# LiMeng95/MultiPoseNet.pytorch

Hardware: AMD Instinct MI355X
Metric: images/sec (train fwd+bwd) ResNet101 480x480 bs=32/GPU (higher is better)
Workload: dtype bf16; 1 GPU; R101 full posenet (keypoint+detection) train step: fwd + MSE/focal losses + bwd + Adam, 480x480, 32 images/GPU, bf16 MFMA / fp32 accumulate / fp32 master weights; global_batch=32, parallelism=dp1, loss_log=asynchronous (set_lazy_log), launch=recorded launch list re-issued per step (replay.py), 87 replays, optimizer_update=Adam in one launch after backward

## Files before the change

include/mpn.h:

```cpp
#ifndef MPN_H_
#define MPN_H_
#include <stdint.h>

#ifdef __cplusplus
extern "C" {
#endif

#define MPN_F32 0
#define MPN_BF16 1
#define MPN_F16 2

#define MPN_E_BADARG (-2)
#define MPN_E_UNSUPPORTED (-3)

typedef struct MpnConvParams {
    const void* x;
    const void* w;
    void* y;
    const float* bias;
    const float* scale;
    const void* res;
    const uint8_t* res_mask;
    float* stats;
    int64_t x_sB, x_sH, x_sW;
// ... 82 lines not shown
int mpn_conv_wgrad_kernel_name(const MpnWgradParams* p, char* buf, int cap);

int mpn_reduce_partials(const float* ws, int chunks, int64_t n, float* dst, int accumulate, void* stream);

int mpn_cast_f32_to_bf16(const float* src, void* dst, int64_t n, void* stream);
int mpn_cast_f32(const float* src, void* dst, int64_t n, int dtype, void* stream);
int mpn_weight_transpose(const float* w, void* wt, int Cout, int RS, int Cin, int Cout_pad,
                         int dtype, void* stream);
int mpn_weight_transpose_batched(const float* arena, void* dst, const int64_t* table, int nlayers, int64_t nblocks,
                                 int dtype, void* stream);
int mpn_weight_pad_k(const float* w, void* dst, int Cout, int K, int Kpad, int dtype, void* stream);
int mpn_stem_pack_weight(const float* w, void* packed, int Cout, int dtype, void* stream);
int mpn_stem_unpack_wgrad(const float* dpacked, float* dw, int Cout, void* stream);
int mpn_stem_pack_image(const float* img, int64_t sB, int64_t sC, int64_t sH, int64_t sW, void* dst,
                        int B, int H, int W, int dtype, void* stream);

int mpn_bn_finalize_train(const float* stats, int tiles, int C, int64_t count, const float* gamma,
                          const float* beta, float* running_mean, float* running_var, float momentum,
                          float eps, float* mean, float* invstd, float* scale, float* shift, void* stream);
int mpn_bn_finalize_eval(int C, const float* gamma, const float* beta, const float* running_mean,
                         const float* running_var, float eps, float* mean, float* invstd,
                         float* scale, float* shift, void* stream);
int mpn_bn_act_forward(const void* y, const void* res, void* z, const float* scale, const float* shift,
                       int64_t P, int C, int Cs, int relu, int dtype, uint8_t* mask, void* stream);
int mpn_bn_bwd_reduce(const void* dz, const void* z, const void* y, const float* mean, const float* invstd,
                      const float* mask_scale, const float* mask_shift, float* partial, int chunks, int64_t P, int C, int Cs, int relu, int dtype, void* stream);
int mpn_bn_bwd_finalize(const float* partial, int chunks, int C, int64_t count, const float* gamma, const float* mean,
                        const float* invstd, int train, float* dgamma, float* dbeta, float* coef, void* stream);
int mpn_bn_bwd_apply(const void* dz, const void* z, const void* y, const float* k1, const float* k2, const float* k3,
                     const float* mask_scale, const float* mask_shift, void* dy, void* dres, int dres_accumulate, int64_t P, int C, int Cs, int relu, int dtype,
                     const uint8_t* mask, void* stream);
int mpn_bn_bwd_chunks(int64_t P, int Cs, int dtype);

int mpn_maxpool3x3s2_forward(const void* x, void* y, uint8_t* idx, int B, int H, int W, int Cs,
                             int Ho, int Wo, int dtype, void* stream);
int mpn_maxpool3x3s2_backward(const void* dy, const uint8_t* idx, void* dx, int B, int H, int W, int Cs,
                              int Ho, int Wo, int dtype, void* stream);
int mpn_upsample_nearest_backward(const void* dfine, void* dcoarse, int B, int Hf, int Wf, int Hc, int Wc,
                                  int Cs, int accumulate, int dtype, void* stream);
int mpn_upsample_nearest_slice(const void* src, void* dst, int B, int Hs, int Ws, int Cs_src,
                               int Ho, int Wo, int Cs_dst, int c_off, int dtype, void* stream);
int mpn_upsample_nearest_slice_backward(const void* ddst, void* dsrc, int B, int Hs, int Ws, int Cs_src,
                                        int Ho, int Wo, int Cs_dst, int c_off, int dtype, void* stream);
int mpn_export_f32(const void* src, int src_dtype, float* dst, int B, int Hs, int Ws, int Cs, int C,
                   int Ho, int Wo, int64_t dst_sB, int64_t dst_sP, void* stream);
int mpn_import_grad(const float* ddst, int64_t ddst_sB, int64_t ddst_sP, void* dsrc, int dst_dtype,
                    int B, int Hs, int Ws, int Cs, int C, int Ho, int Wo, void* stream);
int mpn_nchw_to_nhwc_f32(const float* src, int64_t sB, int64_t sC, int64_t sH, int64_t sW, float* dst,
                         int B, int C, int H, int W, void* stream);
int mpn_det_pack(const void* src, int src_dtype, float* dst, int B, int64_t HW, int Cs, int C, int64_t dst_sB, void* stream);
int mpn_det_unpack(const float* ddst, void* dsrc, int dst_dtype, int B, int64_t HW, int Cs, int C, int64_t dst_sB, void* stream);
int mpn_relu_forward(const void* x, void* y, int64_t n, int dtype, void* stream);
int mpn_relu_backward(const void* dz, const void* z, void* dx, int64_t n, int accumulate, int dtype, void* stream);
int mpn_add_inplace(void* dst, const void* src, int64_t n, int dtype, void* stream);
int mpn_channel_sum(const void* dy, int dy_dtype, int64_t P, int C, int Cs, float* partial, int chunks, void* stream);
int mpn_channel_sum_chunks(int64_t P, int Cs, int dtype);
int mpn_colsum_rows(const void* dy, int dy_dtype, int64_t P, int C, int Cs, float* db, void* stream);

int mpn_mse_heatmap_forward(const float* const* preds, const int64_t* pred_sP, const float* gt, const float* wgt,
                            int64_t npix, float* partial, int chunks, float* out, void* stream);
int mpn_mse_heatmap_backward(const float* const* preds, float* const* dpreds, const int64_t* pred_sP,
                             const int64_t* dpred_sP, const int32_t* pred_C, const float* gt, const float* wgt,
                             int64_t npix, const float* gscale, void* stream);
int mpn_mse_chunks(int64_t npix);
int mpn_mse_train_blocks(int B, int H, int W);
int mpn_mse_heatmap_train(const float* const* levels, void* const* dlevels, const int32_t* level_Cs, int dtype,
// ... 131 lines not shown
```

multiposenet/pytorch_amd/_lib.py:

```python
import ctypes
import os
import subprocess

import torch

_HERE = os.path.dirname(os.path.abspath(__file__))
LIB_PATH = os.path.join(_HERE, "libmpn_hip.so")
CSRC = os.path.join(_HERE, "csrc")

F32, BF16, F16 = 0, 1, 2


class MpnError(RuntimeError):
    pass


class ConvParams(ctypes.Structure):
    _fields_ = [
        ("x", ctypes.c_void_p), ("w", ctypes.c_void_p), ("y", ctypes.c_void_p),
        ("bias", ctypes.c_void_p), ("scale", ctypes.c_void_p), ("res", ctypes.c_void_p), ("res_mask", ctypes.c_void_p),
        ("stats", ctypes.c_void_p),
        ("x_sB", ctypes.c_int64), ("x_sH", ctypes.c_int64), ("x_sW", ctypes.c_int64),
        ("y_sB", ctypes.c_int64), ("y_sP", ctypes.c_int64),
        ("res_sB", ctypes.c_int64), ("res_sP", ctypes.c_int64),
# ... 45 lines not shown
    "mpn_resize": (_i, [_vp, _i64, _i64, _i64, _i, _i, _i, _vp, _i, _i, _i, ctypes.c_double, ctypes.c_double, _vp]),
    "mpn_prn_build_maps": (_i, [_vp, _vp, _vp, _vp, _i, _i, _i, ctypes.c_double, _vp, _vp, _vp, _vp, _vp]),
    "mpn_prn_scores": (_i, [_vp, _vp, _i, _i, _i, _i, _vp, _vp, _vp]),
    "mpn_prn_scores_compact": (_i, [_vp, _vp, _i, _i, _i, _i, _i, _vp, _vp, _vp, _vp, _vp, _vp]),
    "mpn_prn_match_host": (_i, [_i, _vp, _vp, _vp, _vp, _vp, _vp, _vp, _i, _vp, _i, _i, _vp, _vp]),
    "mpn_conv_stats_tiles": (_i, [_PC]),
    "mpn_conv_kernel_name": (_i, [_PC, ctypes.c_char_p, _i]),
    "mpn_conv_forward": (_i, [_PC, _vp]),
    "mpn_debug_wgrad_prof": (_i, [_vp]),
    "mpn_debug_igemm_prof": (_i, [_vp]),
    "mpn_conv_wgrad_chunks": (_i, [_PW]),
    "mpn_conv_wgrad_seg_plan": (_i, [_PW]),
    "mpn_conv_wgrad": (_i, [_PW, _vp]),
    "mpn_conv_wgrad_partials": (_i, [_PW, _vp]),
    "mpn_conv_wgrad_reduce": (_i, [_PW, _vp]),
    "mpn_conv_wgrad_kernel_id": (_i, [_PW]),
    "mpn_conv_wgrad_kernel_name": (_i, [_PW, ctypes.c_char_p, _i]),
    "mpn_reduce_partials": (_i, [_vp, _i, _i64, _vp, _i, _vp]),
    "mpn_cast_f32_to_bf16": (_i, [_vp, _vp, _i64, _vp]),
    "mpn_cast_f32": (_i, [_vp, _vp, _i64, _i, _vp]),
    "mpn_weight_transpose": (_i, [_vp, _vp, _i, _i, _i, _i, _i, _vp]),
    "mpn_weight_transpose_batched": (_i, [_vp, _vp, _vp, _i, _i64, _i, _vp]),
    "mpn_weight_pad_k": (_i, [_vp, _vp, _i, _i, _i, _i, _vp]),
    "mpn_stem_pack_weight": (_i, [_vp, _vp, _i, _i, _vp]),
    "mpn_stem_unpack_wgrad": (_i, [_vp, _vp, _i, _vp]),
    "mpn_stem_pack_image": (_i, [_vp, _i64, _i64, _i64, _i64, _vp, _i, _i, _i, _i, _vp]),
    "mpn_bn_finalize_train": (_i, [_vp, _i, _i, _i64, _vp, _vp, _vp, _vp, _f, _f, _vp, _vp, _vp, _vp, _vp]),
    "mpn_bn_finalize_eval": (_i, [_i, _vp, _vp, _vp, _vp, _f, _vp, _vp, _vp, _vp, _vp]),
    "mpn_bn_act_forward": (_i, [_vp, _vp, _vp, _vp, _vp, _i64, _i, _i, _i, _i, _vp, _vp]),
    "mpn_bn_bwd_reduce": (_i, [_vp, _vp, _vp, _vp, _vp, _vp, _vp, _vp, _i, _i64, _i, _i, _i, _i, _vp]),
    "mpn_bn_bwd_finalize": (_i, [_vp, _i, _i, _i64, _vp, _vp, _vp, _i, _vp, _vp, _vp, _vp]),
    "mpn_bn_bwd_apply": (_i, [_vp, _vp, _vp, _vp, _vp, _vp, _vp, _vp, _vp, _vp, _i, _i64, _i, _i, _i, _i, _vp, _vp]),
    "mpn_bn_bwd_chunks": (_i, [_i64, _i, _i]),
    "mpn_maxpool3x3s2_forward": (_i, [_vp, _vp, _vp, _i, _i, _i, _i, _i, _i, _i, _vp]),
    "mpn_maxpool3x3s2_backward": (_i, [_vp, _vp, _vp, _i, _i, _i, _i, _i, _i, _i, _vp]),
    "mpn_upsample_nearest_backward": (_i, [_vp, _vp, _i, _i, _i, _i, _i, _i, _i, _i, _vp]),
    "mpn_upsample_nearest_slice": (_i, [_vp, _vp, _i, _i, _i, _i, _i, _i, _i, _i, _i, _vp]),
    "mpn_upsample_nearest_slice_backward": (_i, [_vp, _vp, _i, _i, _i, _i, _i, _i, _i, _i, _i, _vp]),
    "mpn_export_f32": (_i, [_vp, _i, _vp, _i, _i, _i, _i, _i, _i, _i, _i64, _i64, _vp]),
    "mpn_import_grad": (_i, [_vp, _i64, _i64, _vp, _i, _i, _i, _i, _i, _i, _i, _i, _vp]),
    "mpn_nchw_to_nhwc_f32": (_i, [_vp, _i64, _i64, _i64, _i64, _vp, _i, _i, _i, _i, _vp]),
    "mpn_det_pack": (_i, [_vp, _i, _vp, _i, _i64, _i, _i, _i64, _vp]),
    "mpn_det_unpack": (_i, [_vp, _vp, _i, _i, _i64, _i, _i, _i64, _vp]),
    "mpn_relu_forward": (_i, [_vp, _vp, _i64, _i, _vp]),
    "mpn_relu_backward": (_i, [_vp, _vp, _vp, _i64, _i, _i, _vp]),
    "mpn_add_inplace": (_i, [_vp, _vp, _i64, _i, _vp]),
    "mpn_channel_sum": (_i, [_vp, _i, _i64, _i, _i, _vp, _i, _vp]),
    "mpn_colsum_rows": (_i, [_vp, _i, _i64, _i, _i, _vp, _vp]),
    "mpn_channel_sum_chunks": (_i, [_i64, _i, _i]),
    "mpn_mse_chunks": (_i, [_i64]),
    "mpn_mse_heatmap_forward": (_i, [_vp, _vp, _vp, _vp, _i64, _vp, _i, _vp, _vp]),
    "mpn_mse_heatmap_backward": (_i, [_vp, _vp, _vp, _vp, _vp, _vp, _vp, _i64, _vp, _vp]),
    "mpn_mse_train_blocks": (_i, [_i, _i, _i]),
    "mpn_mse_heatmap_train": (_i, [_vp, _vp, _vp, _i, _vp, _vp, _i64, _i64, _i64, _i, _i, _i, _vp, _vp, _i, _vp, _vp]),
    "mpn_focal_blocks": (_i, [_i]),
    "mpn_focal_forward": (_i, [_vp, _vp, _vp, _vp, _i, _i, _i, _vp, _vp, _vp, _vp]),
    "mpn_focal_backward": (_i, [_vp, _vp, _vp, _vp, _i, _i, _i, _vp, _vp, _vp, _vp, _vp]),
    "mpn_focal_mc_blocks": (_i, [_i]),
    "mpn_focal_forward_mc": (_i, [_vp, _vp, _vp, _vp, _i, _i, _i, _i, _vp, _vp, _vp, _vp, _vp]),
    "mpn_focal_backward_mc": (_i, [_vp, _vp, _vp, _vp, _i, _i, _i, _i, _vp, _vp, _vp, _vp, _vp]),
    "mpn_class_max": (_i, [_vp, _i, _i, _i, _vp, _vp, _vp]),
    "mpn_sigmoid_forward": (_i, [_vp, _vp, _i64, _vp]),
    "mpn_gather_dets": (_i, [_vp, _vp, _i, _vp, _vp, _vp]),
    "mpn_sigmoid_backward": (_i, [_vp, _vp, _vp, _i64, _vp]),
    "mpn_add_softmax_rows": (_i, [_vp, _i64, _vp, _vp, _i, _i, _i, _vp]),
    "mpn_softmax_rows_backward": (_i, [_vp, _vp, _vp, _i64, _vp, _i, _i, _vp]),
# ... 113 lines not shown
```

multiposenet/pytorch_amd/csrc/bn.hip:

```cpp
#include "common.h"
#include <stdlib.h>

namespace {

template <typename T> struct Geo {
    static constexpr int V = Vec16<T>::N;
    int G, GB, lanes, g, pl, c0;
    __device__ __forceinline__ Geo(int Cs) {
        G = Cs / V;
        GB = G < 256 ? G : 256;
        lanes = 256 / GB;
        g = blockIdx.y * GB + (threadIdx.x % GB);
        pl = threadIdx.x / GB;
        c0 = g * V;
    }
};

template <int V>
__device__ __forceinline__ void load_coef(const float* __restrict__ p, int c0, int C, float (&out)[V], float fill) {
#pragma unroll
    for (int k = 0; k < V; k += 4) {
        if (p != nullptr && c0 + k + 3 < C) {
            const float4 t = *reinterpret_cast<const float4*>(p + c0 + k);
            out[k] = t.x; out[k + 1] = t.y; out[k + 2] = t.z; out[k + 3] = t.w;
// ... 211 lines not shown
    load_coef<V>(k3p, q.c0, C, k3, 0.f);
    const bool bits = relu && mask != nullptr;
    const bool remask = relu && !bits && z == nullptr;
    float sc[V], sf[V];
    if (remask) { load_coef<V>(mscale, q.c0, C, sc, 0.f); load_coef<V>(mshift, q.c0, C, sf, 0.f); }
    const bool need_y = ((dy != nullptr) && (k2p != nullptr)) || remask;
    const long p0 = (long)blockIdx.x * q.lanes * iters + q.pl;
    for (int it = 0; it < iters; ++it) {
        const long p = p0 + (long)it * q.lanes;
        if (p >= P) break;
        const long off = p * Cs + q.c0;
        Vec16<T> d, o, x, out, r;
        d.load(dz + off);
        if (need_y) x.load(y + off);
        if (relu && !remask && !bits) o.load(z + off);
        unsigned mb = 0;
        if (bits) mb = mask[p * q.G + q.g];
        if (dres && dres_acc) r.load(dres + off);
#pragma unroll
        for (int k = 0; k < V; ++k) {
            float gk = d.v[k];
            if (remask) o.v[k] = x.v[k] * sc[k] + sf[k];
            if (bits) o.v[k] = ((mb >> k) & 1u) ? 1.f : 0.f;
            if (relu && !(o.v[k] > 0.f)) gk = 0.f;
            const bool live = q.c0 + k < C;
            out.v[k] = live ? (k1[k] * gk + (k2p ? k2[k] * x.v[k] : 0.f) + k3[k]) : 0.f;
            if (dres) r.v[k] = (dres_acc ? r.v[k] : 0.f) + (live ? gk : 0.f);
        }
        if (dy) out.store(dy + off);
        if (dres) r.store(dres + off);
    }
}

inline int geo_lanes(int Cs, int V) { const int G = Cs / V; return 256 / (G < 256 ? G : 256); }
inline int geo_yblocks(int Cs, int V) { const int G = Cs / V; return G <= 256 ? 1 : G / 256; }
inline bool geo_ok(int Cs, int V) { const int G = Cs / V; return Cs % V == 0 && G > 0 && (G & (G - 1)) == 0; }

inline int pick_iters(long P, int lanes) {
    static const long blocks = mpn_tune("MPN_BN_BLOCKS", 8192);
    long it = P / ((long)lanes * blocks);
    if (it < 1) it = 1;
    if (it > 32) it = 32;
    return (int)it;
}
inline int reduce_chunk(long P, int lanes) {
    long c = P / 512;
    const long lo = (long)lanes * 4, hi = 4096;
    if (c < lo) c = lo;
    if (c > hi) c = hi;
    return (int)((c + lanes - 1) / lanes * lanes);
}

}

extern "C" int mpn_bn_finalize_train(const float* stats, int tiles, int C, int64_t count, const float* gamma,
                                     const float* beta, float* running_mean, float* running_var, float momentum,
                                     float eps, float* mean, float* invstd, float* scale, float* shift, void* stream) {
    MPN_CHECK_ARG(stats && tiles > 0 && C > 0 && count > 0 && mean && invstd && scale && shift);
    hipLaunchKernelGGL(bn_finalize_train_kernel, dim3((C + 3) / 4), dim3(256), 0, (hipStream_t)stream, stats, tiles, C,
                       (double)count, gamma, beta, running_mean, running_var, momentum, eps, mean, invstd, scale, shift);
    return mpn_launch_status();
}

extern "C" int mpn_bn_finalize_eval(int C, const float* gamma, const float* beta, const float* running_mean,
                                    const float* running_var, float eps, float* mean, float* invstd,
                                    float* scale, float* shift, void* stream) {
// ... 31 lines not shown
    const int chunk = reduce_chunk(P, geo_lanes(Cs, V));
    MPN_CHECK_ARG(chunks == (int)((P + chunk - 1) / chunk));
    dim3 grid((unsigned)chunks, (unsigned)geo_yblocks(Cs, V));
    MPN_DISPATCH_T(dtype, hipLaunchKernelGGL((bn_bwd_reduce_kernel<T>), grid, dim3(256), 0, (hipStream_t)stream, (const T*)dz, (const T*)z,
                           (const T*)y, mean, invstd, mask_scale, mask_shift, partial, (long)P, C, Cs, relu, chunk));
    return mpn_launch_status();
}

extern "C" int mpn_bn_bwd_finalize(const float* partial, int chunks, int C, int64_t count, const float* gamma, const float* mean,
                                   const float* invstd, int train, float* dgamma, float* dbeta, float* coef, void* stream) {
    MPN_CHECK_ARG(partial && chunks > 0 && C > 0 && count > 0);
    MPN_CHECK_ARG(!coef || (mean && invstd));
    hipLaunchKernelGGL(bn_bwd_finalize_kernel, dim3((C + 3) / 4), dim3(256), 0, (hipStream_t)stream, partial, chunks, C,
                       (double)count, gamma, mean, invstd, train, dgamma, dbeta, coef);
    return mpn_launch_status();
}

extern "C" int mpn_bn_bwd_apply(const void* dz, const void* z, const void* y, const float* k1, const float* k2, const float* k3,
                                const float* mask_scale, const float* mask_shift, void* dy, void* dres, int dres_accumulate, int64_t P, int C, int Cs, int relu, int dtype,
                                const uint8_t* mask, void* stream) {
    MPN_CHECK_ARG(dz && (dy || dres) && P > 0 && C > 0 && Cs >= C);
    MPN_CHECK_ARG(!dy || k1);
    MPN_CHECK_ARG(!(dy && k2) || y);
    MPN_CHECK_ARG(!relu || z || mask || (mask_scale && mask_shift && y));
    const int V = dtype == MPN_F32 ? 4 : 8;
    MPN_CHECK_ARG(geo_ok(Cs, V) && C % 4 == 0);
    const int lanes = geo_lanes(Cs, V), iters = pick_iters(P, lanes);
    dim3 grid((unsigned)((P + (long)lanes * iters - 1) / ((long)lanes * iters)), (unsigned)geo_yblocks(Cs, V));
    MPN_DISPATCH_T(dtype, hipLaunchKernelGGL((bn_bwd_apply_kernel<T>), grid, dim3(256), 0, (hipStream_t)stream, (const T*)dz, (const T*)z,
                           (const T*)y, k1, k2, k3, mask_scale, mask_shift, (T*)dy, (T*)dres, dres_accumulate, (long)P, C, Cs, relu, iters,
                           (const unsigned char*)mask));
    return mpn_launch_status();
}
```

multiposenet/pytorch_amd/engine.py:

```python
import ctypes
import os

import torch

from . import ops
from ._lib import MpnError, call, gpu_op
from .ops import Act, round_up


class Ctx(object):

    def __init__(self, train):
        self.train = train
        self.tape = []
        self.grads = {}
        self.keep = []
        self.out_grads = {}
        self.wt = {}
        self.wt_buf = None
        self.uses = {}
        self.bn_train_ran = False
        self.side_keep = []
        self.wt_ready = None
        self.bnb = {}
# ... 22 lines not shown
        return self.grads.pop(id(act), None)


def num_classes(cm):
    cout = cm.output.weight.shape[0]
    if cout % 9 != 0 or cout == 0 or getattr(cm, "num_anchors", 9) != 9:
        raise MpnError("classificationModel: the output convolution has %d channels; the detector needs 9 anchors x K classes" % cout)
    return cout // 9


def _geom(layer):
    w = layer.weight
    if w.dim() == 2:
        return w.shape[0], w.shape[1], 1, 1, 1, 0
    return w.shape[0], w.shape[1], w.shape[2], w.shape[3], layer.stride[0], layer.padding[0]


class Engine(object):
    def __init__(self, model):
        self.m = model
        self._drop_calls = 0
        self._side = None
        self._wt_plan_cache = None
        self.overlap_wgrad = os.environ.get("MPN_SIDE_STREAM", "1") != "0"
        self.pyramid_towers = os.environ.get("MPN_PYRAMID_TOWERS", "1") != "0"
        self.fuse_bn_stats = os.environ.get("MPN_BN_FUSED_STATS", "1") != "0"
        self.fold_bn = os.environ.get("MPN_FOLD_BN", "1") != "0"
        self.fuse_bn_finalize = os.environ.get("MPN_BN_FUSED_FINALIZE", "1") != "0"
        self.det_pyramid_side = int(os.environ.get("MPN_DET_PYRAMID_SIDE", "2"))
        self.bn_mask_bits = os.environ.get("MPN_BN_MASK_BITS", "1") != "0"
        self.defer_shortcut_grad = os.environ.get("MPN_DEFER_SHORTCUT_GRAD", "1") != "0"
        self.virtual_concat = os.environ.get("MPN_VIRTUAL_CONCAT", "1") != "0"
        self.conv2_classes = os.environ.get("MPN_CONV2_CLASSES", "1") != "0"

    def side_stream(self, device):
        if not self.overlap_wgrad or device.type != "cuda":
            return None
        if self._side is None:
            self._side = torch.cuda.Stream(device=device)
        return self._side

    def _on_side(self, ctx, device, keep, fn, torch_ops=False, done_event=False):
        side = self.side_stream(device)
        if side is None:
            fn()
            return None
        ctx.side_keep.append(keep)
        ev = torch.cuda.Event()
        gpu_op(ev.record, torch.cuda.current_stream(device))
        gpu_op(side.wait_event, ev)
        if torch_ops:
            with torch.cuda.stream(side):
                fn()
        else:
            ops.push_stream(side)
            try:
                fn()
            finally:
                ops.pop_stream()
        if not done_event:
            return None
        done = torch.cuda.Event()
        gpu_op(done.record, side)
        return done

    @property
# ... 221 lines not shown
            raise MpnError("pyramid convolution: gradient missing for some levels")
        if act == 1:
            fd, fy = ops.seg_flat(dys), ops.seg_flat(ys)
            if fd is not None and fy is not None and fd.numel() == fy.numel():
                out = ops.alloc_seg(ys, ys[0].C, dys[0].t.dtype)
                call("mpn_relu_backward", ops.ptr(fd), ops.ptr(fy), ops.ptr(out[0].seg[0]), fy.numel(), 0, ops.dtype_code(fy.dtype), ops.stream_ptr())
                dys = out
            else:
                dys = [ops.relu_backward(d, y) for d, y in zip(dys, ys)]
        pyr = []

        def wgrad(dw, db, i):
            if i == 0:
                pyr[:] = ops.conv_wgrad_seg(xs, dys, dw, O, R, S, pad, db=db)
            return pyr[1] if pyr[0] else ops.conv_wgrad(xs[i], dys[i], dw, O, R, S, 1, pad, db=db)
        self._param_grads(ctx, layer, dys, (xs, dys), wgrad)
        if any(x.needs_grad for x in xs):
            wt = self.w_t(ctx, layer)
            grouped = ops.seg_flat(xs) is not None
            if grouped and ctx.grad_of(xs[0]) is None:
                gs = ops.alloc_seg(xs, xs[0].C, xs[0].t.dtype)
                for x, g in zip(xs, gs):
                    ctx.set_grad(x, g)
                existed = [False] * len(xs)
            else:
                pairs = [ctx.gbuf(x) for x in xs]
                gs, existed = [g for g, _ in pairs], [e for _, e in pairs]
            if all(existed) or not any(existed):
                ops.conv_forward_seg(dys, wt, I, R, S, pad, mode=1, cin=wt.shape[3], outs=gs, accumulate=existed[0])
            else:
                for d, x, g, e in zip(dys, xs, gs, existed):
                    ops.conv_forward(d, wt, I, R, S, 1, pad, mode=1, out_hw=(x.H, x.W), cin=wt.shape[3], out=g, accumulate=e)

    def bn(self, ctx, y, stats, layer, relu, res=None, tag=""):
        train_stats = layer.training
        want_mask = bool(self.bn_mask_bits and ctx.train and relu and res is not None)
        if train_stats:
            momentum = layer.momentum if layer.momentum is not None else 0.1
            if isinstance(stats, ops.BNState):
                st = stats
            else:
                st = ops.bn_finalize_train(stats, y.P, layer.weight.data, layer.bias.data, layer.running_mean, layer.running_var,
                                           momentum, layer.eps)
            ctx.bn_train_ran = True
        else:
            st = ops.bn_finalize_eval(layer.weight.data, layer.bias.data, layer.running_mean, layer.running_var, layer.eps)
        z = ops.bn_act(y, st, relu, res=res, tag=tag, want_mask=want_mask)
        if ctx.train:
            z.needs_grad = bool(y.needs_grad or layer.weight.requires_grad or layer.bias.requires_grad
                                or (res is not None and res.needs_grad))
            if z.needs_grad:
                self._note_use(ctx, layer.weight)
                self._note_use(ctx, layer.bias)
                if res is not None and res.needs_grad:
                    res.cons += 1
                    res.other_cons += 1
                wants_stats = bool(train_stats or layer.weight.requires_grad or layer.bias.requires_grad)
                z.bn_src = (y, st, relu, res is not None, wants_stats, layer, train_stats)
                ctx.tape.append(lambda: self._bn_bwd(ctx, y, z, st, layer, relu, res, train_stats))
        return z

    @staticmethod
    def _bnb_args(fused):
        if fused is None:
            return {}
        if isinstance(fused, str) or (fused.dim() == 2 and fused.shape[0] == 3):
            return {"coef": fused}
        return {"partial": fused}

    def _bn_bwd(self, ctx, y, z, st, layer, relu, res, train_stats):
        dz = ctx.pop_grad(z)
        wg, bg = layer.weight.requires_grad, layer.bias.requires_grad
        if dz is None:
            self._param_grads(ctx, layer, None)
            if res is not None and res.needs_grad:
                res.cons -= 1
            return
        ar = self.m._arena
        dres, dres_acc = None, False
# ... 260 lines not shown
            img = img.float()
        packed = torch.empty((B, Hp, Wp, 4), dtype=self.cdt, device=img.device)
        call("mpn_stem_pack_image", ops.ptr(img), img.stride(0), img.stride(1), img.stride(2), img.stride(3), ops.ptr(packed),
             B, H, W, ops.dtype_code(self.cdt), ops.stream_ptr())
        xa = Act(packed, 4)
        w = f.conv1.weight
        wp = torch.empty((64, 7, 32), dtype=self.cdt, device=img.device)
        call("mpn_stem_pack_weight", ops.ptr(self.m._arena.data_seg(w)), ops.ptr(wp), 64, ops.dtype_code(self.cdt), ops.stream_ptr())
        Ho, Wo = ops.conv_out_hw(H, W, 7, 7, 2, 3)
        geom = (Hp, Wp, Hp * Wp * 4, Wp * 4, 4)
        bn_train = f.bn1.training
        if self.fold_bn and not ctx.train and not bn_train:
            bst = ops.bn_finalize_eval(f.bn1.weight.data, f.bn1.bias.data, f.bn1.running_mean, f.bn1.running_var, f.bn1.eps)
            z, _ = ops.conv_forward(xa, wp, 64, 7, 1, 2, 0, cin=32, x_geom=geom, out_hw=(Ho, Wo), scale=bst.scale, bias=bst.shift, act=1)
            return self.maxpool(ctx, z)
        y, st = ops.conv_forward(xa, wp, 64, 7, 1, 2, 0, cin=32, x_geom=geom, out_hw=(Ho, Wo), want_stats=bn_train,
                                 bn_fin=self._bn_fin(f.bn1) if bn_train else None)
        if ctx.train and w.requires_grad:
            y.needs_grad = True
            self._note_use(ctx, w)

            def bwd():
                dy = ctx.pop_grad(y)
                if dy is None:
                    return self._param_grads(ctx, f.conv1, None)
                dwp = torch.empty((64, 7, 32), dtype=torch.float32, device=img.device)

                def wgrad(dw, db, i):
                    call("mpn_fill_f32", ops.ptr(dwp), 0.0, dwp.numel(), ops.stream_ptr())
                    ops.conv_wgrad(xa, dy, dwp, 64, 7, 1, 2, 0, cin=32, x_geom=geom)
                    call("mpn_stem_unpack_wgrad", ops.ptr(dwp), ops.ptr(dw), 64, ops.stream_ptr())
                self._param_grads(ctx, f.conv1, (dy,), (xa, dy, dwp), wgrad)
            ctx.tape.append(bwd)
        z = self.bn(ctx, y, st, f.bn1, True)
        return self.maxpool(ctx, z)

    def conv_bn(self, ctx, x, conv, bn, relu, res=None):
        if self.fold_bn and not ctx.train and not bn.training:
            st = ops.bn_finalize_eval(bn.weight.data, bn.bias.data, bn.running_mean, bn.running_var, bn.eps)
            O, I, R, S, stride, pad = _geom(conv)
            act = (3 if res is not None else 1) if relu else 0
            y, _ = ops.conv_forward(x, self.w_fwd(conv), O, R, S, stride, pad, scale=st.scale, bias=st.shift, act=act,
                                    res=res, res_mode=1 if res is not None else 0)
            return y
        y, s = self.conv(ctx, x, conv, stats=bn.training, bn=bn)
        return self.bn(ctx, y, s, bn, relu, res=res)

    def bottleneck(self, ctx, x, blk):
        z1 = self.conv_bn(ctx, x, blk.conv1, blk.bn1, True)
        z2 = self.conv_bn(ctx, z1, blk.conv2, blk.bn2, True)
        sc = self.conv_bn(ctx, x, blk.downsample[0], blk.downsample[1], False) if len(blk.downsample) > 0 else x
        return self.conv_bn(ctx, z2, blk.conv3, blk.bn3, True, res=sc)

    def backbone(self, ctx, img):
        f = self.m.fpn
        c = self.stem(ctx, img)
        feats = []
        for layer in (f.layer1, f.layer2, f.layer3, f.layer4):
            for blk in layer:
                c = self.bottleneck(ctx, c, blk)
            feats.append(c)
        return feats

    def det_pyramid(self, ctx, c3, c4, c5):
        f = self.m.fpn

        def coarse(h):
            h["p6"], _ = self.conv(ctx, c5, f.conv6)
# ... 160 lines not shown
```

multiposenet/pytorch_amd/ops.py:

```python
import ctypes
import os

import torch

from . import _lib
from ._lib import BF16, F16, F32, ConvParams, WgradParams, call


def round_up(v, m):
    return (v + m - 1) // m * m


def dtype_code(dt):
    if dt == torch.float32:
        return F32
    if dt == torch.bfloat16:
        return BF16
    if dt == torch.float16:
        return F16
    raise _lib.MpnError("unsupported dtype %s" % dt)


_STREAM_OVERRIDE = []

# ... 665 lines not shown
                 chunks, P, C, Cs, 1 if relu else 0, dc, stream_ptr())
        coef = torch.empty((3, C), dtype=torch.float32, device=dev) if train else None
        call("mpn_bn_bwd_finalize", ptr(part), chunks, C, P, ptr(gamma), ptr(st.mean), ptr(st.invstd), 1 if train else 0,
             ptr(dgamma), ptr(dbeta), ptr(coef), stream_ptr())
        if train:
            k1, k2, k3 = coef[0], coef[1], coef[2]
    dy = None
    if want_dy or dres is not None:
        if want_dy:
            dy = Act(torch.empty_like(y.t), C)
        bits = z.mask if (relu and not remask) else None
        call("mpn_bn_bwd_apply", ptr(dz.t), ptr(z.t) if (relu and not remask and bits is None) else None, ptr(y.t), ptr(k1), ptr(k2), ptr(k3),
             ptr(st.scale) if remask else None, ptr(st.shift) if remask else None,
             ptr(dy.t) if dy is not None else None, ptr(dres.t) if dres is not None else None,
             1 if dres_acc else 0, P, C, Cs, 1 if relu else 0, dc, ptr(bits), stream_ptr())
    return dy


def maxpool_forward(x, needs_grad=False):
    Ho, Wo = (x.H + 2 - 3) // 2 + 1, (x.W + 2 - 3) // 2 + 1
    y = Act(torch.empty((x.B, Ho, Wo, x.Cs), dtype=x.t.dtype, device=x.t.device), x.C, needs_grad)
    idx = torch.empty((x.B, Ho, Wo, x.Cs), dtype=torch.uint8, device=x.t.device) if needs_grad else None
    call("mpn_maxpool3x3s2_forward", ptr(x.t), ptr(y.t), ptr(idx), x.B, x.H, x.W, x.Cs, Ho, Wo, dtype_code(x.t.dtype), stream_ptr())
    return y, idx


def maxpool_backward(dy, idx, x_like):
    dx = Act(torch.empty_like(x_like.t), x_like.C)
    call("mpn_maxpool3x3s2_backward", ptr(dy.t), ptr(idx), ptr(dx.t), x_like.B, x_like.H, x_like.W, x_like.Cs, dy.H, dy.W,
         dtype_code(dy.t.dtype), stream_ptr())
    return dx


def upsample_backward(dfine, dcoarse, accumulate):
    call("mpn_upsample_nearest_backward", ptr(dfine.t), ptr(dcoarse.t), dfine.B, dfine.H, dfine.W, dcoarse.H, dcoarse.W,
         dfine.Cs, 1 if accumulate else 0, dtype_code(dfine.t.dtype), stream_ptr())


def upsample_slice(src, dst, c_off):
    call("mpn_upsample_nearest_slice", ptr(src.t), ptr(dst.t), src.B, src.H, src.W, src.Cs, dst.H, dst.W, dst.Cs, c_off,
         dtype_code(src.t.dtype), stream_ptr())


def upsample_slice_backward(ddst, dsrc, c_off):
    call("mpn_upsample_nearest_slice_backward", ptr(ddst.t), ptr(dsrc.t), dsrc.B, dsrc.H, dsrc.W, dsrc.Cs, ddst.H, ddst.W,
         ddst.Cs, c_off, dtype_code(dsrc.t.dtype), stream_ptr())


def export_f32(src, C, Ho, Wo):
    out = torch.empty((src.B, Ho, Wo, C), dtype=torch.float32, device=src.t.device)
    call("mpn_export_f32", ptr(src.t), dtype_code(src.t.dtype), ptr(out), src.B, src.H, src.W, src.Cs, C, Ho, Wo,
         Ho * Wo * C, C, stream_ptr())
    return out.permute(0, 3, 1, 2)


def import_grad(g_nchw, like, dtype):
    B, C, Ho, Wo = g_nchw.shape
    g = g_nchw.permute(0, 2, 3, 1)
    if g.stride(3) != 1 or g.stride(1) != Wo * g.stride(2):
        g = g.contiguous()
    d = Act(torch.empty((like.B, like.H, like.W, like.Cs), dtype=dtype, device=like.t.device), like.C)
    call("mpn_import_grad", ptr(g), g.stride(0), g.stride(2), ptr(d.t), dtype_code(dtype), like.B, like.H, like.W, like.Cs,
         like.C, Ho, Wo, stream_ptr())
    return d


# ... 163 lines not shown
```

Measured before the change: 889.8 images/sec.

## Fuse stem BN+ReLU with 3x3 maxpool in forward and backward

Adds kernels that apply the stem BatchNorm affine and ReLU while computing the 3x3/s2 maxpool, so the full-resolution post-BN activation is never written. The backward pass scatters pooled gradients through the stored argmax indices inside the BN backward reduce and apply kernels, which removes the separate maxpool backward and its full-resolution gradient tensor. This cuts several full-resolution memory passes at 240x240x64. In exchange the forward recomputes BN for overlapping pool windows, and the backward gathers up to four pooled neighbours per pixel and re-derives the ReLU mask from y and the BN coefficients.

```diff
diff --git a/include/mpn.h b/include/mpn.h
--- a/include/mpn.h
+++ b/include/mpn.h
@@ -138,6 +138,17 @@
                      const uint8_t* mask, void* stream);
 int mpn_bn_bwd_chunks(int64_t P, int Cs, int dtype);
 
+int mpn_stem_bn_act_pool_forward(const void* y, void* pooled, uint8_t* idx, uint8_t* mask, const float* scale,
+                                 const float* shift, int B, int H, int W, int C, int Cs, int Ho, int Wo, int dtype,
+                                 void* stream);
+int mpn_stem_pool_bn_bwd_reduce(const void* dpooled, const uint8_t* idx, const void* y, const float* mean,
+                                const float* invstd, const float* mask_scale, const float* mask_shift,
+                                const uint8_t* mask, float* partial, int chunks, int B, int H, int W, int C, int Cs,
+                                int Ho, int Wo, int dtype, void* stream);
+int mpn_stem_pool_bn_bwd_apply(const void* dpooled, const uint8_t* idx, const void* y, const float* k1, const float* k2,
+                               const float* k3, const float* mask_scale, const float* mask_shift, const uint8_t* mask,
+                               void* dy, int B, int H, int W, int C, int Cs, int Ho, int Wo, int dtype, void* stream);
+
 int mpn_maxpool3x3s2_forward(const void* x, void* y, uint8_t* idx, int B, int H, int W, int Cs,
                              int Ho, int Wo, int dtype, void* stream);
 int mpn_maxpool3x3s2_backward(const void* dy, const uint8_t* idx, void* dx, int B, int H, int W, int Cs,
diff --git a/multiposenet/pytorch_amd/_lib.py b/multiposenet/pytorch_amd/_lib.py
--- a/multiposenet/pytorch_amd/_lib.py
+++ b/multiposenet/pytorch_amd/_lib.py
@@ -101,6 +101,9 @@
     "mpn_bn_bwd_finalize": (_i, [_vp, _i, _i, _i64, _vp, _vp, _vp, _i, _vp, _vp, _vp, _vp]),
     "mpn_bn_bwd_apply": (_i, [_vp, _vp, _vp, _vp, _vp, _vp, _vp, _vp, _vp, _vp, _i, _i64, _i, _i, _i, _i, _vp, _vp]),
     "mpn_bn_bwd_chunks": (_i, [_i64, _i, _i]),
+    "mpn_stem_bn_act_pool_forward": (_i, [_vp, _vp, _vp, _vp, _vp, _vp, _i, _i, _i, _i, _i, _i, _i, _i, _vp]),
+    "mpn_stem_pool_bn_bwd_reduce": (_i, [_vp, _vp, _vp, _vp, _vp, _vp, _vp, _vp, _vp, _i, _i, _i, _i, _i, _i, _i, _i, _i, _vp]),
+    "mpn_stem_pool_bn_bwd_apply": (_i, [_vp, _vp, _vp, _vp, _vp, _vp, _vp, _vp, _vp, _vp, _i, _i, _i, _i, _i, _i, _i, _i, _vp]),
     "mpn_maxpool3x3s2_forward": (_i, [_vp, _vp, _vp, _i, _i, _i, _i, _i, _i, _i, _vp]),
     "mpn_maxpool3x3s2_backward": (_i, [_vp, _vp, _vp, _i, _i, _i, _i, _i, _i, _i, _vp]),
     "mpn_upsample_nearest_backward": (_i, [_vp, _vp, _i, _i, _i, _i, _i, _i, _i, _i, _vp]),
diff --git a/multiposenet/pytorch_amd/csrc/bn.hip b/multiposenet/pytorch_amd/csrc/bn.hip
--- a/multiposenet/pytorch_amd/csrc/bn.hip
+++ b/multiposenet/pytorch_amd/csrc/bn.hip
@@ -267,6 +267,227 @@
     }
 }
 
+
+template <int V> struct IdxVec;
+template <> struct IdxVec<8> {
+    uint2 t;
+    __device__ __forceinline__ void load(const uint8_t* p) { t = *reinterpret_cast<const uint2*>(p); }
+    __device__ __forceinline__ void store(uint8_t* p) const { *reinterpret_cast<uint2*>(p) = t; }
+    __device__ __forceinline__ unsigned get(int k) const { return ((k < 4 ? t.x : t.y) >> ((k & 3) * 8)) & 0xffu; }
+    __device__ __forceinline__ void set(const int (&b)[8]) {
+        t.x = (unsigned)b[0] | ((unsigned)b[1] << 8) | ((unsigned)b[2] << 16) | ((unsigned)b[3] << 24);
+        t.y = (unsigned)b[4] | ((unsigned)b[5] << 8) | ((unsigned)b[6] << 16) | ((unsigned)b[7] << 24);
+    }
+};
+template <> struct IdxVec<4> {
+    unsigned t;
+    __device__ __forceinline__ void load(const uint8_t* p) { t = *reinterpret_cast<const unsigned*>(p); }
+    __device__ __forceinline__ void store(uint8_t* p) const { *reinterpret_cast<unsigned*>(p) = t; }
+    __device__ __forceinline__ unsigned get(int k) const { return (t >> (k * 8)) & 0xffu; }
+    __device__ __forceinline__ void set(const int (&b)[4]) {
+        t = (unsigned)b[0] | ((unsigned)b[1] << 8) | ((unsigned)b[2] << 16) | ((unsigned)b[3] << 24);
+    }
+};
+
+template <typename T>
+__global__ void __launch_bounds__(256) stem_bn_act_pool_fwd_kernel(const T* __restrict__ y, T* __restrict__ out, uint8_t* __restrict__ idx,
+                                                                   unsigned char* __restrict__ mask, const float* __restrict__ scale,
+                                                                   const float* __restrict__ shift, int B, int H, int W, int C, int Cs,
+                                                                   int Ho, int Wo) {
+    constexpr int V = Vec16<T>::N;
+    const unsigned G = Cs / V;
+    const unsigned i = blockIdx.x * blockDim.x + threadIdx.x;
+    if (i >= (unsigned)B * Ho * Wo * G) return;
+    const unsigned g = i % G;
+    unsigned pix = i / G;
+    const int wo = (int)(pix % Wo); pix /= Wo;
+    const int ho = (int)(pix % Ho);
+    const int b = (int)(pix / Ho);
+    const int c0 = g * V;
+    float sc[V], sf[V];
+    load_coef<V>(scale, c0, C, sc, 0.f);
+    load_coef<V>(shift, c0, C, sf, 0.f);
+    float best[V]; int bi[V];
+#pragma unroll
+    for (int k = 0; k < V; ++k) { best[k] = -INFINITY; bi[k] = 0; }
+    bool first = true;
+    for (int r = 0; r < 3; ++r) {
+        const int h = ho * 2 - 1 + r;
+        if ((unsigned)h >= (unsigned)H) continue;
+        for (int s = 0; s < 3; ++s) {
+            const int w = wo * 2 - 1 + s;
+            if ((unsigned)w >= (unsigned)W) continue;
+            const long p = ((long)b * H + h) * W + w;
+            Vec16<T> a; a.load(y + p * Cs + c0);
+            unsigned bits = 0;
+#pragma unroll
+            for (int k = 0; k < V; ++k) {
+                float x = a.v[k] * sc[k] + sf[k];
+                x = fmaxf(x, 0.f);
+                const float v = Elem<T>::round((c0 + k < C) ? x : 0.f);
+                bits |= (v > 0.f ? 1u : 0u) << k;
+                if (first || v > best[k]) { best[k] = v; bi[k] = r * 3 + s; }
+            }
+            first = false;
+            if (mask && r >= 1 && s >= 1) mask[p * G + g] = (unsigned char)bits;
+        }
+    }
+    Vec16<T> o;
+#pragma unroll
+    for (int k = 0; k < V; ++k) o.v[k] = best[k];
+    o.store(out + (long)i * V);
+    if (idx) {
+        IdxVec<V> t; t.set(bi);
+        t.store(idx + (long)i * V);
+    }
+}
+
+template <typename T>
+struct StemPoolGather {
+    static constexpr int V = Vec16<T>::N;
+    Vec16<T> v[4];
+    IdxVec<V> ix[4];
+    unsigned tap[4];
+    bool ok[4];
+    __device__ __forceinline__ void issue(const T* __restrict__ dpool, const uint8_t* __restrict__ idx, unsigned p,
+                                          int H, int W, int Ho, int Wo, unsigned G, unsigned g) {
+        const int w = (int)(p % (unsigned)W);
+        const unsigned t = p / (unsigned)W;
+        const int h = (int)(t % (unsigned)H);
+        const int b = (int)(t / (unsigned)H);
+        const int ho0 = h >> 1, wo0 = w >> 1;
+        const bool vh = (h & 1) && ho0 + 1 < Ho, vw = (w & 1) && wo0 + 1 < Wo;
+        const unsigned r0 = (h & 1) ? 2 : 1, s0 = (w & 1) ? 2 : 1;
+        const long o00 = ((((long)b * Ho + ho0) * Wo + wo0) * G + g) * V;
+        const long dw = vw ? (long)G * V : 0, dh = vh ? (long)Wo * G * V : 0;
+        const long o[4] = {o00, o00 + dw, o00 + dh, o00 + dh + dw};
+        tap[0] = r0 * 3 + s0; tap[1] = r0 * 3; tap[2] = s0; tap[3] = 0;
+        ok[0] = true; ok[1] = vw; ok[2] = vh; ok[3] = vh && vw;
+#pragma unroll
+        for (int j = 0; j < 4; ++j) { v[j].load(dpool + o[j]); ix[j].load(idx + o[j]); }
+    }
+    __device__ __forceinline__ void finish(Vec16<T>& d) const {
+        float acc[V];
+#pragma unroll
+        for (int k = 0; k < V; ++k) acc[k] = 0.f;
+#pragma unroll
+        for (int j = 0; j < 4; ++j) {
+#pragma unroll
+            for (int k = 0; k < V; ++k) acc[k] = (ok[j] && ix[j].get(k) == tap[j]) ? acc[k] + v[j].v[k] : acc[k];
+        }
+#pragma unroll
+        for (int k = 0; k < V; ++k) d.v[k] = Elem<T>::round(acc[k]);
+    }
+};
+
+template <typename T>
+__global__ void __launch_bounds__(256) stem_pool_bn_bwd_reduce_kernel(const T* __restrict__ dpool, const uint8_t* __restrict__ idx,
+                                                                      const T* __restrict__ y, const float* __restrict__ mean,
+                                                                      const float* __restrict__ invstd, const float* __restrict__ mscale,
+                                                                      const float* __restrict__ mshift, const unsigned char* __restrict__ mask,
+                                                                      float* __restrict__ partial, int H, int W, int Ho, int Wo, long P,
+                                                                      int C, int Cs, int chunk_pix) {
+    constexpr int V = Vec16<T>::N;
+    __shared__ float sh[256][2 * V + 1];
+    const Geo<T> q(Cs);
+    const long p_begin = (long)blockIdx.x * chunk_pix;
+    long p_end = p_begin + chunk_pix; if (p_end > P) p_end = P;
+    float s1[V], s2[V], mu[V], is[V], sc[V], sf[V];
+    load_coef<V>(mean, q.c0, C, mu, 0.f);
+    load_coef<V>(invstd, q.c0, C, is, 0.f);
+    const bool remask = mask == nullptr;
+    if (remask) { load_coef<V>(mscale, q.c0, C, sc, 0.f); load_coef<V>(mshift, q.c0, C, sf, 0.f); }
+#pragma unroll
+    for (int k = 0; k < V; ++k) { s1[k] = 0.f; s2[k] = 0.f; }
+    for (long p = p_begin + q.pl; p < p_end; p += 2 * q.lanes) {
+        const bool two = p + q.lanes < p_end;
+        const long pp[2] = {p, two ? p + q.lanes : p};
+        Vec16<T> x[2];
+        unsigned mb[2] = {0, 0};
+        StemPoolGather<T> gt[2];
+#pragma unroll
+        for (int u = 0; u < 2; ++u) {
+            x[u].load(y + pp[u] * Cs + q.c0);
+            if (!remask) mb[u] = mask[pp[u] * q.G + q.g];
+            gt[u].issue(dpool, idx, (unsigned)pp[u], H, W, Ho, Wo, q.G, q.g);
+        }
+#pragma unroll
+        for (int u = 0; u < 2; ++u) {
+            if (u == 1 && !two) break;
+            Vec16<T> d, o;
+            gt[u].finish(d);
+#pragma unroll
+            for (int k = 0; k < V; ++k) {
+                float gk = d.v[k];
+                if (remask) o.v[k] = x[u].v[k] * sc[k] + sf[k];
+                else o.v[k] = ((mb[u] >> k) & 1u) ? 1.f : 0.f;
+                if (!(o.v[k] > 0.f)) gk = 0.f;
+                s1[k] += gk;
+                s2[k] += gk * ((x[u].v[k] - mu[k]) * is[k]);
+            }
+        }
+    }
+#pragma unroll
+    for (int k = 0; k < V; ++k) { sh[threadIdx.x][k] = s1[k]; sh[threadIdx.x][V + k] = s2[k]; }
+    __syncthreads();
+    if (q.pl == 0) {
+        for (int l = 1; l < q.lanes; ++l) {
+#pragma unroll
+            for (int k = 0; k < V; ++k) {
+                s1[k] += sh[threadIdx.x + l * q.GB][k];
+                s2[k] += sh[threadIdx.x + l * q.GB][V + k];
+            }
+        }
+#pragma unroll
+        for (int k = 0; k < V; ++k) {
+            const int c = q.c0 + k;
+            if (c < C) *reinterpret_cast<float2*>(partial + ((long)blockIdx.x * C + c) * 2) = make_float2(s1[k], s2[k]);
+        }
+    }
+}
+
+template <typename T>
+__global__ void __launch_bounds__(256) stem_pool_bn_bwd_apply_kernel(const T* __restrict__ dpool, const uint8_t* __restrict__ idx,
+                                                                     const T* __restrict__ y, const float* __restrict__ k1p,
+                                                                     const float* __restrict__ k2p, const float* __restrict__ k3p,
+                                                                     const float* __restrict__ mscale, const float* __restrict__ mshift,
+                                                                     const unsigned char* __restrict__ mask, T* __restrict__ dy,
+                                                                     int H, int W, int Ho, int Wo, long P, int C, int Cs, int iters) {
+    constexpr int V = Vec16<T>::N;
+    const Geo<T> q(Cs);
+    float k1[V], k2[V], k3[V];
+    load_coef<V>(k1p, q.c0, C, k1, 0.f);
+    load_coef<V>(k2p, q.c0, C, k2, 0.f);
+    load_coef<V>(k3p, q.c0, C, k3, 0.f);
+    const bool remask = mask == nullptr;
+    float sc[V], sf[V];
+    if (remask) { load_coef<V>(mscale, q.c0, C, sc, 0.f); load_coef<V>(mshift, q.c0, C, sf, 0.f); }
+    const bool need_y = (k2p != nullptr) || remask;
+    const long p0 = (long)blockIdx.x * q.lanes * iters + q.pl;
+    for (int it = 0; it < iters; ++it) {
+        const long p = p0 + (long)it * q.lanes;
+        if (p >= P) break;
+        const long off = p * Cs + q.c0;
+        Vec16<T> d, o, x, out;
+        if (need_y) x.load(y + off);
+        unsigned mb = 0;
+        if (!remask) mb = mask[p * q.G + q.g];
+        StemPoolGather<T> gt;
+        gt.issue(dpool, idx, (unsigned)p, H, W, Ho, Wo, q.G, q.g);
+        gt.finish(d);
+#pragma unroll
+        for (int k = 0; k < V; ++k) {
+            float gk = d.v[k];
+            if (remask) o.v[k] = x.v[k] * sc[k] + sf[k];
+            else o.v[k] = ((mb >> k) & 1u) ? 1.f : 0.f;
+            if (!(o.v[k] > 0.f)) gk = 0.f;
+            const bool live = q.c0 + k < C;
+            out.v[k] = live ? (k1[k] * gk + (k2p ? k2[k] * x.v[k] : 0.f) + k3[k]) : 0.f;
+        }
+        out.store(dy + off);
+    }
+}
+
 inline int geo_lanes(int Cs, int V) { const int G = Cs / V; return 256 / (G < 256 ? G : 256); }
 inline int geo_yblocks(int Cs, int V) { const int G = Cs / V; return G <= 256 ? 1 : G / 256; }
 inline bool geo_ok(int Cs, int V) { const int G = Cs / V; return Cs % V == 0 && G > 0 && (G & (G - 1)) == 0; }
@@ -364,3 +585,58 @@
                            (const unsigned char*)mask));
     return mpn_launch_status();
 }
+
+static bool stem_pool_geo_ok(int B, int H, int W, int C, int Cs, int Ho, int Wo, int dtype) {
+    if (!mpn_dtype_ok(dtype) || B <= 0 || H <= 0 || W <= 0 || C <= 0 || Cs < C) return false;
+    const int V = dtype == MPN_F32 ? 4 : 8;
+    if (!geo_ok(Cs, V) || C % 4 != 0) return false;
+    if (Ho != (H - 1) / 2 + 1 || Wo != (W - 1) / 2 + 1) return false;
+    return (long)B * H * W * (Cs / V) < (1L << 31);
+}
+
+extern "C" int mpn_stem_bn_act_pool_forward(const void* y, void* pooled, uint8_t* idx, uint8_t* mask, const float* scale,
+                                            const float* shift, int B, int H, int W, int C, int Cs, int Ho, int Wo, int dtype,
+                                            void* stream) {
+    MPN_CHECK_ARG(y && pooled && scale && shift);
+    MPN_CHECK_ARG(stem_pool_geo_ok(B, H, W, C, Cs, Ho, Wo, dtype));
+    const int V = dtype == MPN_F32 ? 4 : 8;
+    const long n = (long)B * Ho * Wo * (Cs / V);
+    MPN_DISPATCH_T(dtype, hipLaunchKernelGGL((stem_bn_act_pool_fwd_kernel<T>), dim3((unsigned)((n + 255) / 256)), dim3(256), 0,
+                           (hipStream_t)stream, (const T*)y, (T*)pooled, idx, (unsigned char*)mask, scale, shift, B, H, W, C, Cs, Ho, Wo));
+    return mpn_launch_status();
+}
+
+extern "C" int mpn_stem_pool_bn_bwd_reduce(const void* dpooled, const uint8_t* idx, const void* y, const float* mean,
+                                           const float* invstd, const float* mask_scale, const float* mask_shift,
+                                           const uint8_t* mask, float* partial, int chunks, int B, int H, int W, int C, int Cs,
+                                           int Ho, int Wo, int dtype, void* stream) {
+    MPN_CHECK_ARG(dpooled && idx && y && mean && invstd && partial);
+    MPN_CHECK_ARG(mask || (mask_scale && mask_shift));
+    MPN_CHECK_ARG(stem_pool_geo_ok(B, H, W, C, Cs, Ho, Wo, dtype));
+    const int V = dtype == MPN_F32 ? 4 : 8;
+    const long P = (long)B * H * W;
+    const int chunk = reduce_chunk(P, geo_lanes(Cs, V));
+    MPN_CHECK_ARG(chunks == (int)((P + chunk - 1) / chunk));
+    dim3 grid((unsigned)chunks, (unsigned)geo_yblocks(Cs, V));
+    MPN_DISPATCH_T(dtype, hipLaunchKernelGGL((stem_pool_bn_bwd_reduce_kernel<T>), grid, dim3(256), 0, (hipStream_t)stream,
+                           (const T*)dpooled, idx, (const T*)y, mean, invstd, mask_scale, mask_shift, (const unsigned char*)mask,
+                           partial, H, W, Ho, Wo, P, C, Cs, chunk));
+    return mpn_launch_status();
+}
+
+extern "C" int mpn_stem_pool_bn_bwd_apply(const void* dpooled, const uint8_t* idx, const void* y, const float* k1, const float* k2,
+                                          const float* k3, const float* mask_scale, const float* mask_shift, const uint8_t* mask,
+                                          void* dy, int B, int H, int W, int C, int Cs, int Ho, int Wo, int dtype, void* stream) {
+    MPN_CHECK_ARG(dpooled && idx && dy && k1);
+    MPN_CHECK_ARG(mask || (mask_scale && mask_shift));
+    MPN_CHECK_ARG(!(k2 || !mask) || y);
+    MPN_CHECK_ARG(stem_pool_geo_ok(B, H, W, C, Cs, Ho, Wo, dtype));
+    const int V = dtype == MPN_F32 ? 4 : 8;
+    const long P = (long)B * H * W;
+    const int lanes = geo_lanes(Cs, V), iters = pick_iters(P, lanes);
+    dim3 grid((unsigned)((P + (long)lanes * iters - 1) / ((long)lanes * iters)), (unsigned)geo_yblocks(Cs, V));
+    MPN_DISPATCH_T(dtype, hipLaunchKernelGGL((stem_pool_bn_bwd_apply_kernel<T>), grid, dim3(256), 0, (hipStream_t)stream,
+                           (const T*)dpooled, idx, (const T*)y, k1, k2, k3, mask_scale, mask_shift, (const unsigned char*)mask,
+                           (T*)dy, H, W, Ho, Wo, P, C, Cs, iters));
+    return mpn_launch_status();
+}
diff --git a/multiposenet/pytorch_amd/engine.py b/multiposenet/pytorch_amd/engine.py
--- a/multiposenet/pytorch_amd/engine.py
+++ b/multiposenet/pytorch_amd/engine.py
@@ -78,6 +78,7 @@
         self.defer_shortcut_grad = os.environ.get("MPN_DEFER_SHORTCUT_GRAD", "1") != "0"
         self.virtual_concat = os.environ.get("MPN_VIRTUAL_CONCAT", "1") != "0"
         self.conv2_classes = os.environ.get("MPN_CONV2_CLASSES", "1") != "0"
+        self.stem_fused = os.environ.get("MPN_STEM_FUSED", "1") != "0"
 
     def side_stream(self, device):
         if not self.overlap_wgrad or device.type != "cuda":
@@ -365,19 +366,20 @@
                 for d, x, g, e in zip(dys, xs, gs, existed):
                     ops.conv_forward(d, wt, I, R, S, 1, pad, mode=1, out_hw=(x.H, x.W), cin=wt.shape[3], out=g, accumulate=e)
 
+    def _bn_state(self, ctx, y, stats, layer):
+        if not layer.training:
+            return ops.bn_finalize_eval(layer.weight.data, layer.bias.data, layer.running_mean, layer.running_var, layer.eps)
+        ctx.bn_train_ran = True
+        if isinstance(stats, ops.BNState):
+            return stats
+        momentum = layer.momentum if layer.momentum is not None else 0.1
+        return ops.bn_finalize_train(stats, y.P, layer.weight.data, layer.bias.data, layer.running_mean, layer.running_var,
+                                     momentum, layer.eps)
+
     def bn(self, ctx, y, stats, layer, relu, res=None, tag=""):
         train_stats = layer.training
         want_mask = bool(self.bn_mask_bits and ctx.train and relu and res is not None)
-        if train_stats:
-            momentum = layer.momentum if layer.momentum is not None else 0.1
-            if isinstance(stats, ops.BNState):
-                st = stats
-            else:
-                st = ops.bn_finalize_train(stats, y.P, layer.weight.data, layer.bias.data, layer.running_mean, layer.running_var,
-                                           momentum, layer.eps)
-            ctx.bn_train_ran = True
-        else:
-            st = ops.bn_finalize_eval(layer.weight.data, layer.bias.data, layer.running_mean, layer.running_var, layer.eps)
+        st = self._bn_state(ctx, y, stats, layer)
         z = ops.bn_act(y, st, relu, res=res, tag=tag, want_mask=want_mask)
         if ctx.train:
             z.needs_grad = bool(y.needs_grad or layer.weight.requires_grad or layer.bias.requires_grad
@@ -704,8 +706,34 @@
                     call("mpn_stem_unpack_wgrad", ops.ptr(dwp), ops.ptr(dw), 64, ops.stream_ptr())
                 self._param_grads(ctx, f.conv1, (dy,), (xa, dy, dwp), wgrad)
             ctx.tape.append(bwd)
-        z = self.bn(ctx, y, st, f.bn1, True)
+        bn1 = f.bn1
+        affine = bn1.weight.requires_grad or bn1.bias.requires_grad
+        if self.stem_fused and self.fuse_bn_stats and ctx.train and (y.needs_grad or affine) and (bn_train or affine):
+            return self.bn_relu_pool(ctx, y, st, bn1)
+        z = self.bn(ctx, y, st, bn1, True)
         return self.maxpool(ctx, z)
+
+    def bn_relu_pool(self, ctx, y, stats, layer):
+        train_stats = layer.training
+        st = self._bn_state(ctx, y, stats, layer)
+        p, idx = ops.stem_bn_act_pool(y, st, needs_grad=True)
+        self._note_use(ctx, layer.weight)
+        self._note_use(ctx, layer.bias)
+        wg, bg = layer.weight.requires_grad, layer.bias.requires_grad
+
+        def bwd():
+            dp = ctx.pop_grad(p)
+            if dp is None:
+                return self._param_grads(ctx, layer, None)
+            ar = self.m._arena
+            dy = ops.stem_pool_bn_backward(dp, idx, y, st, layer.weight.data, train_stats,
+                                           dgamma=ar.grad_seg(layer.weight) if wg else None,
+                                           dbeta=ar.grad_seg(layer.bias) if bg else None, want_dy=y.needs_grad)
+            self._param_grads(ctx, layer, None)
+            if y.needs_grad:
+                ctx.set_grad(y, dy)
+        ctx.tape.append(bwd)
+        return p
 
     def conv_bn(self, ctx, x, conv, bn, relu, res=None):
         if self.fold_bn and not ctx.train and not bn.training:
diff --git a/multiposenet/pytorch_amd/ops.py b/multiposenet/pytorch_amd/ops.py
--- a/multiposenet/pytorch_amd/ops.py
+++ b/multiposenet/pytorch_amd/ops.py
@@ -721,6 +721,42 @@
     return dx
 
 
+def stem_bn_act_pool(y, st, needs_grad=False, want_mask=False):
+    Ho, Wo = (y.H + 2 - 3) // 2 + 1, (y.W + 2 - 3) // 2 + 1
+    dev = y.t.device
+    p = Act(torch.empty((y.B, Ho, Wo, y.Cs), dtype=y.t.dtype, device=dev), y.C, needs_grad)
+    idx = torch.empty((y.B, Ho, Wo, y.Cs), dtype=torch.uint8, device=dev) if needs_grad else None
+    if want_mask:
+        p.mask = torch.empty((y.P, y.Cs // (4 if y.t.dtype == torch.float32 else 8)), dtype=torch.uint8, device=dev)
+    call("mpn_stem_bn_act_pool_forward", ptr(y.t), ptr(p.t), ptr(idx), ptr(p.mask), ptr(st.scale), ptr(st.shift),
+         y.B, y.H, y.W, y.C, y.Cs, Ho, Wo, dtype_code(y.t.dtype), stream_ptr())
+    return p, idx
+
+
+def stem_pool_bn_backward(dp, idx, y, st, gamma, train, dgamma=None, dbeta=None, want_dy=True, mask=None):
+    dev = y.t.device
+    C, Cs = y.C, y.Cs
+    dc = dtype_code(y.t.dtype)
+    if not (train or dgamma is not None or dbeta is not None):
+        raise _lib.MpnError("stem_pool_bn_backward: frozen BatchNorm without parameter gradients takes bn_backward")
+    geo = (y.B, y.H, y.W, C, Cs, dp.H, dp.W, dc)
+    msc, msh = (None, None) if mask is not None else (st.scale, st.shift)
+    chunks = call("mpn_bn_bwd_chunks", y.P, Cs, dc)
+    part = workspace(chunks * C * 2 * 4, dev, slot=3)
+    call("mpn_stem_pool_bn_bwd_reduce", ptr(dp.t), ptr(idx), ptr(y.t), ptr(st.mean), ptr(st.invstd), ptr(msc), ptr(msh), ptr(mask),
+         ptr(part), chunks, *geo, stream_ptr())
+    coef = torch.empty((3, C), dtype=torch.float32, device=dev) if train else None
+    call("mpn_bn_bwd_finalize", ptr(part), chunks, C, y.P, ptr(gamma), ptr(st.mean), ptr(st.invstd), 1 if train else 0,
+         ptr(dgamma), ptr(dbeta), ptr(coef), stream_ptr())
+    if not want_dy:
+        return None
+    k1, k2, k3 = (coef[0], coef[1], coef[2]) if train else (st.scale, None, None)
+    dy = Act(torch.empty_like(y.t), C)
+    call("mpn_stem_pool_bn_bwd_apply", ptr(dp.t), ptr(idx), ptr(y.t), ptr(k1), ptr(k2), ptr(k3), ptr(msc), ptr(msh), ptr(mask),
+         ptr(dy.t), *geo, stream_ptr())
+    return dy
+
+
 def upsample_backward(dfine, dcoarse, accumulate):
     call("mpn_upsample_nearest_backward", ptr(dfine.t), ptr(dcoarse.t), dfine.B, dfine.H, dfine.W, dcoarse.H, dcoarse.W,
          dfine.Cs, 1 if accumulate else 0, dtype_code(dfine.t.dtype), stream_ptr())
```

Result: no change. 893.9 images/sec, median of 6 (+0.5%).
